# zhuzhui-2000/mobilesuperresolution

Measured on AMD Instinct MI355X. Metric: HR megapixels/sec (WDSR-B x4, 48x48 LR patches), full training step, higher is better.
Workload: dtype bf16; 1 GPU; WDSR-B x4, 16 blocks / 24 units, 48x48 LR patches, batch 32 per GPU, fwd+L1+bwd+Adam; global_batch=32, parallelism=dp1

## Files before the change

mobilesuperresolution_amd/csrc/sr_abi.hip:

```cpp
#include <algorithm>
#include <cmath>
#include "../../include/sr_hotpath.h"
#include "wdsr_block.h"
#include "wdsr_fwd_rs.h"
#include "wdsr_fwd_stream.h"
#include "wdsr_bwd_rs.h"
#include "wdsr_bwd_pair_lds.h"
#include "wdsr_wgrad_rs.h"
#include "wdsr_ends.h"
#include "wdsr_prep.h"
#include "conv3x3.h"
#include "conv64.h"
#include "conv64_bwd.h"
#include "vsr_recon.h"
#include "vsr_recon_bwd.h"
#include "mv_recon.h"
#include "spynet_conv.h"
#include "nas_block.h"
#include "nas_dw_lc.h"
#include "nas_bwd_fused.h"
#include "flow_warp.h"
#include "metrics.h"
#include "ssim.h"
#include "eval.h"
// ... 298 lines not shown
  if (dtype != SR_DTYPE_BF16) return -1;
  return dispatch_f(F, [&](auto d) {
    return launch_wgrad_saved<decltype(d)::F>(x, dy, tsave, dtsave, wblob, cinit, pa, pb, layers, wgs, N, H, W, x_ls, dy_ls, side_ls,
                                                  w_ls, c_ls, (hipStream_t)stream);
  });
}

extern "C" int sr_wdsr_block_slab_sizes(int F, int* slab_a, int* slab_b) {
  if (!slab_a || !slab_b) return -2;
  return dispatch_f(F, [&](auto d) {
    typedef BwdCfg<typename decltype(d)::Cfg> B;
    *slab_a = B::SLAB_A;
    *slab_b = B::SLAB_B;
    return 0;
  });
}

extern "C" int sr_wdsr_block_fwd(const void* x, void* y, const void* wblob, const float* cinit, int N, int H,
                                 int W, int F, int dtype, sr_stream_t stream) {
  if (!x || !y || !wblob || !cinit || N <= 0 || H <= 0 || W <= 0 || N > 65535) return -2;
  return dispatch_ft(F, dtype, [&](auto d, auto t) {
    return launch_block_fwd<decltype(t), decltype(d)::F>(x, y, wblob, cinit, N, H, W, (hipStream_t)stream);
  });
}

namespace {
template <typename E> dim3 tile_grid(int N, int H, int W, int* tiles_x) {
  *tiles_x = (W + E::TW - 1) / E::TW;
  return dim3(*tiles_x * ((H + E::TH - 1) / E::TH), N);
}
#define SR_DISPATCH_TF(CALL)                                                     \
  if (F == 24 && dtype == SR_DTYPE_BF16) { CALL(__bf16, 24) }                    \
  else if (F == 24 && dtype == SR_DTYPE_F32) { CALL(float, 24) }                 \
  else if (F == 32 && dtype == SR_DTYPE_BF16) { CALL(__bf16, 32) }               \
  else if (F == 32 && dtype == SR_DTYPE_F32) { CALL(float, 32) }                 \
  else return -1;
#define SR_DISPATCH_R(CALL, T, F_)                                               \
  if (R == 4) { CALL(T, F_, 4) } else if (R == 2) { CALL(T, F_, 2) } else if (R == 3) { CALL(T, F_, 3) } else return -1;
}

extern "C" int sr_head_fwd(const float* x, void* y, const void* wblob, float mean, int N, int H, int W, int F,
                           int dtype, sr_stream_t stream) {
  if (!x || !y || !wblob || N <= 0 || H <= 0 || W <= 0 || N > 65535) return -2;
  hipStream_t st = (hipStream_t)stream;
#define CALL(T, F_) { typedef EndsCfg<F_, 4> E; int tx; dim3 g = tile_grid<E>(N, H, W, &tx); \
    hipLaunchKernelGGL((sr_head_fwd_kernel<T, F_>), g, dim3(256), 0, st, x, (T*)y, (const T*)wblob, mean, H, W, tx); }
  SR_DISPATCH_TF(CALL)
#undef CALL
  SR_HIP_CHECK_LAUNCH();
  return 0;
}

extern "C" int sr_tail_fwd(const void* feat, const float* x, float* out, const void* wblob, float mean, int N,
                           int H, int W, int F, int R, int dtype, sr_stream_t stream) {
  if (!feat || !x || !out || !wblob || N <= 0 || H <= 0 || W <= 0 || N > 65535) return -2;
  hipStream_t st = (hipStream_t)stream;
#define CALLR(T, F_, R_) { typedef EndsCfg<F_, R_> E; int tx; dim3 g = tile_grid<E>(N, H, W, &tx); \
    hipLaunchKernelGGL((sr_tail_fwd_kernel<T, F_, R_>), g, dim3(SR_TAIL_FWD_THREADS), 0, st, (const T*)feat, x, out, (const T*)wblob, mean, H, W, tx); }
#define CALL(T, F_) SR_DISPATCH_R(CALLR, T, F_)
  SR_DISPATCH_TF(CALL)
#undef CALL
#undef CALLR
  SR_HIP_CHECK_LAUNCH();
  return 0;
}

namespace {
template <int LOSS>
int tail_bwd_data_t(const float* dout, const float* hr, float gscale, void* dfeat, const void* wblob, int N, int H, int W, int F,
                    int R, int dtype, hipStream_t st) {
  const LossIn li{hr, gscale};
#define CALLR(T, F_, R_) { typedef EndsCfg<F_, R_> E; int tx; dim3 g = tile_grid<E>(N, H, W, &tx); \
    hipLaunchKernelGGL((sr_tail_bwd_data_kernel<T, F_, R_, LOSS>), g, dim3(256), 0, st, dout, (T*)dfeat, (const T*)wblob, H, W, tx, li); }
#define CALL(T, F_) SR_DISPATCH_R(CALLR, T, F_)
  SR_DISPATCH_TF(CALL)
#undef CALL
#undef CALLR
  SR_HIP_CHECK_LAUNCH();
  return 0;
}
template <int LOSS>
int tail_wgrad_t(const float* dout, const float* hr, float gscale, float* loss_part, const void* feat, const float* x, float mean,
                 float* partial, int wgs, int N, int H, int W, int F, int R, int dtype, hipStream_t st) {
  const LossIn li{hr, gscale};
#define CALLR(T, F_, R_) { typedef EndsCfg<F_, R_> E; const int tx = (W + E::TW - 1) / E::TW, tpi = tx * ((H + E::TH - 1) / E::TH); \
    hipLaunchKernelGGL((sr_tail_wgrad_kernel<T, F_, R_, LOSS>), dim3(wgs), dim3(896), 0, st, dout, (const T*)feat, x, mean, partial, N, H, W, tx, tpi, li, loss_part); }
#define CALL(T, F_) SR_DISPATCH_R(CALLR, T, F_)
  SR_DISPATCH_TF(CALL)
#undef CALL
#undef CALLR
  SR_HIP_CHECK_LAUNCH();
  return 0;
}
template <int LOSS>
int tail_bwd_t(const float* dout, const float* hr, float gscale, float* loss_part, const void* feat, const float* x, float mean,
               const void* wblob, void* dfeat, float* partial, int wgs, int N, int H, int W, int F, int R, hipStream_t st) {
  const LossIn li{hr, gscale};
  typedef __bf16 TB;
#define CALLR(T, F_, R_) { typedef EndsCfg<F_, R_> E; const int tx = (W + E::TW - 1) / E::TW, tpi = tx * ((H + E::TH - 1) / E::TH); \
    hipLaunchKernelGGL((sr_tail_bwd_kernel<T, F_, R_, LOSS>), dim3(wgs), dim3(896), 0, st, dout, (const T*)feat, x, mean, (const T*)wblob, (T*)dfeat, partial, N, H, W, tx, tpi, li, loss_part); }
  if (F == 24) { SR_DISPATCH_R(CALLR, TB, 24) } else if (F == 32) { SR_DISPATCH_R(CALLR, TB, 32) } else return -1;
#undef CALLR
  SR_HIP_CHECK_LAUNCH();
  return 0;
}
}

extern "C" int sr_tail_bwd_data(const float* dout, void* dfeat, const void* wblob, int N, int H, int W, int F,
                                int R, int dtype, sr_stream_t stream) {
  if (!dout || !dfeat || !wblob || N <= 0 || H <= 0 || W <= 0 || N > 65535) return -2;
  return tail_bwd_data_t<0>(dout, nullptr, 0.f, dfeat, wblob, N, H, W, F, R, dtype, (hipStream_t)stream);
}

extern "C" int sr_tail_wgrad(const float* dout, const void* feat, const float* x, float mean, float* partial,
                             int wgs, int N, int H, int W, int F, int R, int dtype, sr_stream_t stream) {
  if (!dout || !feat || !x || !partial || wgs <= 0 || N <= 0 || H <= 0 || W <= 0) return -2;
  return tail_wgrad_t<0>(dout, nullptr, 0.f, nullptr, feat, x, mean, partial, wgs, N, H, W, F, R, dtype, (hipStream_t)stream);
}

extern "C" int sr_tail_bwd(const float* dout, const void* feat, const float* x, float mean, const void* wblob,
                          void* dfeat, float* partial, int wgs, int N, int H, int W, int F, int R, int dtype,
                          sr_stream_t stream) {
  if (!dout || !feat || !x || !wblob || !dfeat || !partial || wgs <= 0 || N <= 0 || H <= 0 || W <= 0) return -2;
  if (dtype != SR_DTYPE_BF16) return -1;
  return tail_bwd_t<0>(dout, nullptr, 0.f, nullptr, feat, x, mean, wblob, dfeat, partial, wgs, N, H, W, F, R, (hipStream_t)stream);
}

extern "C" int sr_tail_bwd_loss(const float* sr, const float* hr, int loss_kind, float gscale, float* loss_part, const void* feat,
                                const float* x, float mean, const void* wblob, void* dfeat, float* partial, int wgs, int N,
                                int H, int W, int F, int R, int dtype, sr_stream_t stream) {
  if (!sr || !hr || !loss_part || !feat || !x || !wblob || !dfeat || !partial || wgs <= 0 || N <= 0 || H <= 0 || W <= 0 || N > 65535)
    return -2;
  if (loss_kind != 1 && loss_kind != 2) return -1;
  hipStream_t st = (hipStream_t)stream;
  if (dtype == SR_DTYPE_BF16)
    return loss_kind == 1 ? tail_bwd_t<1>(sr, hr, gscale, loss_part, feat, x, mean, wblob, dfeat, partial, wgs, N, H, W, F, R, st)
                          : tail_bwd_t<2>(sr, hr, gscale, loss_part, feat, x, mean, wblob, dfeat, partial, wgs, N, H, W, F, R, st);
  int rc = loss_kind == 1 ? tail_bwd_data_t<1>(sr, hr, gscale, dfeat, wblob, N, H, W, F, R, dtype, st)
                          : tail_bwd_data_t<2>(sr, hr, gscale, dfeat, wblob, N, H, W, F, R, dtype, st);
  if (rc) return rc;
  return loss_kind == 1 ? tail_wgrad_t<1>(sr, hr, gscale, loss_part, feat, x, mean, partial, wgs, N, H, W, F, R, dtype, st)
                        : tail_wgrad_t<2>(sr, hr, gscale, loss_part, feat, x, mean, partial, wgs, N, H, W, F, R, dtype, st);
}

extern "C" int sr_tail_train(const float* hr, int loss_kind, float gscale, float* loss_part, const void* feat, const float* x,
                             float mean, const void* wblob, void* dfeat, float* partial, int wgs, int N, int H, int W, int F,
                             int R, int dtype, sr_stream_t stream) {
  if (!hr || !loss_part || !feat || !x || !wblob || !dfeat || !partial || wgs <= 0 || N <= 0 || H <= 0 || W <= 0 || N > 65535)
    return -2;
  if (dtype != SR_DTYPE_BF16 || R != 4 || (F != 24 && F != 32) || (loss_kind != 1 && loss_kind != 2)) return -1;
  hipStream_t st = (hipStream_t)stream;
  const LossIn li{hr, gscale};
  typedef __bf16 TB;
#define CALL(F_, LOSS) { typedef EndsCfg<F_, 4> E; const int tx = (W + E::TW - 1) / E::TW, tpi = tx * ((H + E::TH - 1) / E::TH); \
    hipLaunchKernelGGL((sr_tail_train_kernel<TB, F_, 4, LOSS>), dim3(wgs), dim3(896), 0, st, (const TB*)feat, x, mean, (const TB*)wblob, (TB*)dfeat, partial, N, H, W, tx, tpi, li, loss_part); }
  if (F == 24) { if (loss_kind == 1) CALL(24, 1) else CALL(24, 2) }
  else { if (loss_kind == 1) CALL(32, 1) else CALL(32, 2) }
#undef CALL
  SR_HIP_CHECK_LAUNCH();
  return 0;
}

extern "C" int sr_head_wgrad(const void* dy0, const float* x, float mean, float* partial, int wgs, int N, int H,
                             int W, int F, int dtype, sr_stream_t stream) {
  if (!dy0 || !x || !partial || wgs <= 0 || N <= 0 || H <= 0 || W <= 0) return -2;
  hipStream_t st = (hipStream_t)stream;
#define CALL(T, F_) { typedef EndsCfg<F_, 4> E; const int tx = (W + E::TW - 1) / E::TW, tpi = tx * ((H + E::TH - 1) / E::TH); \
    hipLaunchKernelGGL((sr_head_wgrad_kernel<T, F_>), dim3(wgs), dim3(576), 0, st, (const T*)dy0, x, mean, partial, N, H, W, tx, tpi); }
  SR_DISPATCH_TF(CALL)
#undef CALL
  SR_HIP_CHECK_LAUNCH();
  return 0;
}

namespace {
struct C3Grid { int tx, tpi; dim3 grid; };
inline C3Grid c3_grid(int N, int H, int W) {
  C3Grid g;
  g.tx = (W + C3Cfg::TW - 1) / C3Cfg::TW;
  g.tpi = g.tx * ((H + C3Cfg::TH - 1) / C3Cfg::TH);
  g.grid = dim3(g.tpi, N);
  return g;
}
template <typename T> C3WarpSrc<T> c3_warp_src(const sr_c3_warp_t* w) {
  C3WarpSrc<T> s{};
  if (w) { s.frame = w->frame; s.state = (const T*)w->state; s.flow = w->flow; s.frame_bs = w->frame_bs; s.flow_bs = w->flow_bs; s.x0_save = (T*)w->x0_save; }
  return s;
}
template <typename T>
int c3_fwd_t(const void* x, const void* res, void* y, const void* w, int N, int H, int W, int CI, int act, hipStream_t st,
             const sr_c3_warp_t* warp = nullptr, C3Dir dir = C3Dir{0, 0}) {
  const C3Grid g = c3_grid(N, H, W);
  const dim3 blk(64 * C3Cfg::NPT_O);
  const C3WarpSrc<T> ws = c3_warp_src<T>(warp);
#define L(CI_, ONES_, ACT_, ADD_) hipLaunchKernelGGL((c3_fwd_kernel<T, CI_, ONES_, ACT_, ADD_>), g.grid, blk, 0, st, (const T*)x, (const T*)res, (T*)y, (const T*)w, H, W, g.tx, ws, dir)
  if (warp) {
    if (CI != 32 || act != 2 || res) return -1;
    hipLaunchKernelGGL((c3_fwd_kernel<T, 32, 27, 2, false, true>), g.grid, blk, 0, st, (const T*)nullptr, (const T*)nullptr, (T*)y,
                       (const T*)w, H, W, g.tx, ws, dir);
  } else if (CI == 32 && act == 2 && !res) L(32, 27, 2, false);
  else if (CI == 24 && act == 2 && !res) L(24, 24, 2, false);
  else if (CI == 24 && act == 1 && !res) L(24, 24, 1, false);
  else if (CI == 24 && act == 0 && res) L(24, 24, 0, true);
  else if (CI == 24 && act == 0 && !res) L(24, 24, 0, false);
  else return -1;
#undef L
  SR_HIP_CHECK_LAUNCH();
  return 0;
}
template <typename T>
int c3_bwd_t(const void* dA, const void* A, const void* add, void* dx, const void* w, int N, int H, int W, int CI, int act,
             hipStream_t st, C3Dir dir = C3Dir{0, 0}) {
  const C3Grid g = c3_grid(N, H, W);
  const dim3 blk(64 * C3Cfg::NPT_O);
#define L(CI_, ACT_, ADD_) hipLaunchKernelGGL((c3_bwd_data_kernel<T, CI_, ACT_, ADD_>), g.grid, blk, 0, st, (const T*)dA, (const T*)A, (const T*)add, (T*)dx, (const T*)w, H, W, g.tx, dir)
  if (CI == 32 && act == 2 && !add) L(32, 2, false);
  else if (CI == 24 && act == 2 && !add) L(24, 2, false);
  else if (CI == 24 && act == 1 && add) L(24, 1, true);
  else if (CI == 24 && act == 1 && !add) L(24, 1, false);
  else if (CI == 24 && act == 0 && !add) L(24, 0, false);
  else return -1;
#undef L
  SR_HIP_CHECK_LAUNCH();
  return 0;
}
template <typename T>
int c3_wgrad_t(const void* x, const void* dA, const void* A, float* partial, int wgs, int N, int H, int W, int CI, int act,
               hipStream_t st, int layers = 1, long x_ls = 0, long d_ls = 0, long a_ls = 0, long p_ls = 0,
               const sr_c3_warp_t* warp = nullptr, int n_dir = 0) {
  const C3Grid g = c3_grid(N, H, W);
  const C3WarpSrc<T> ws = c3_warp_src<T>(warp);
#define L(CI_, ONES_, ACT_) hipLaunchKernelGGL((c3_wgrad_kernel<T, CI_, ONES_, ACT_>), dim3(wgs, layers), dim3(576), 0, st, (const T*)x, (const T*)dA, (const T*)A, partial, N, H, W, g.tx, g.tpi, x_ls, d_ls, a_ls, p_ls, ws, n_dir)
  if (warp) {
    if (CI != 32 || act != 2 || layers != 1) return -1;
    hipLaunchKernelGGL((c3_wgrad_kernel<T, 32, 27, 2, true>), dim3(wgs, 1), dim3(576), 0, st, (const T*)nullptr, (const T*)dA,
                       (const T*)A, partial, N, H, W, g.tx, g.tpi, x_ls, d_ls, a_ls, p_ls, ws, n_dir);
  } else if (CI == 32 && act == 2) L(32, 27, 2);
  else if (CI == 24 && act == 2) L(24, 24, 2);
  else if (CI == 24 && act == 1) L(24, 24, 1);
  else if (CI == 24 && act == 0) L(24, 24, 0);
  else return -1;
#undef L
  SR_HIP_CHECK_LAUNCH();
  return 0;
}
}

extern "C" int sr_c3_fwd(const void* x, const void* res, void* y, const void* wblob, int N, int H, int W, int CI,
                         int act, int dtype, sr_stream_t stream) {
  if (!x || !y || !wblob || N <= 0 || H <= 0 || W <= 0 || N > 65535) return -2;
  return dtype == SR_DTYPE_BF16 ? c3_fwd_t<__bf16>(x, res, y, wblob, N, H, W, CI, act, (hipStream_t)stream)
                                : c3_fwd_t<float>(x, res, y, wblob, N, H, W, CI, act, (hipStream_t)stream);
}
extern "C" int sr_c3_bwd_data(const void* dA, const void* A, const void* add, void* dx, const void* wblob, int N,
                              int H, int W, int CI, int act, int dtype, sr_stream_t stream) {
  if (!dA || !dx || !wblob || (act != 0 && !A) || N <= 0 || H <= 0 || W <= 0 || N > 65535) return -2;
  if (!A) A = dA;
  return dtype == SR_DTYPE_BF16 ? c3_bwd_t<__bf16>(dA, A, add, dx, wblob, N, H, W, CI, act, (hipStream_t)stream)
                                : c3_bwd_t<float>(dA, A, add, dx, wblob, N, H, W, CI, act, (hipStream_t)stream);
}
extern "C" int sr_c3_wgrad(const void* x, const void* dA, const void* A, float* partial, int wgs, int N, int H,
                           int W, int CI, int act, int dtype, sr_stream_t stream) {
  if (!x || !dA || !partial || (act != 0 && !A) || wgs <= 0 || N <= 0 || H <= 0 || W <= 0) return -2;
  if (!A) A = dA;
  return dtype == SR_DTYPE_BF16 ? c3_wgrad_t<__bf16>(x, dA, A, partial, wgs, N, H, W, CI, act, (hipStream_t)stream)
                                : c3_wgrad_t<float>(x, dA, A, partial, wgs, N, H, W, CI, act, (hipStream_t)stream);
}

template <typename T>
static int c3_trunk_fwd_t(const void* x0, const sr_c3_warp_t* warp, void* acts_, void* mids_, const void* blob_,
                          const long* boff, int nb, int N, int H, int W, int ci0, hipStream_t st, C3Dir dir) {
  const size_t act = (size_t)N * H * W * 24;
  T* acts = (T*)acts_; T* mids = (T*)mids_; const T* blob = (const T*)blob_;
  int rc;
  if ((rc = c3_fwd_t<T>(x0, nullptr, acts, blob + boff[0], N, H, W, ci0, 2, st, warp, dir))) return rc;
  for (int i = 0; i < nb; ++i) {
    if constexpr (sizeof(T) == 2) {
      const C3Grid g = c3_grid(N, H, W);
      if (i + 1 < nb) {
        hipLaunchKernelGGL((c3_resblock2_fwd_kernel<T>), g.grid, dim3(64 * C3Quad::NWAVES), 0, st, acts + i * act, mids + i * act,
                           acts + (i + 1) * act, mids + (i + 1) * act, acts + (i + 2) * act, blob, boff[1 + 2 * i], boff[2 + 2 * i],
                           boff[3 + 2 * i], boff[4 + 2 * i], H, W, g.tx, dir);
        SR_HIP_CHECK_LAUNCH();
        ++i;
        continue;
      }
      hipLaunchKernelGGL((c3_resblock_fwd_kernel<T>), g.grid, dim3(64 * C3Pair::NPT_H), 0, st, acts + i * act, mids + i * act,
                         acts + (i + 1) * act, blob + boff[1 + 2 * i], blob + boff[2 + 2 * i], H, W, g.tx, dir);
      SR_HIP_CHECK_LAUNCH();
      continue;
    }
    if ((rc = c3_fwd_t<T>(acts + i * act, nullptr, mids + i * act, blob + boff[1 + 2 * i], N, H, W, 24, 1, st, nullptr, dir))) return rc;
    if ((rc = c3_fwd_t<T>(mids + i * act, acts + i * act, acts + (i + 1) * act, blob + boff[2 + 2 * i], N, H, W, 24, 0, st, nullptr, dir)))
      return rc;
  }
  return 0;
}
template <typename T>
static int c3_trunk_bwd_t(const void* x0, const sr_c3_warp_t* warp, const void* acts_, const void* mids_, void* ga_, void* gt_,
                          const void* blob_, const long* boff, float* parts, void* dx0, const sr_c3_unpack_t* up, int nb,
                          int wgs, int N, int H, int W, int ci0, hipStream_t st, C3Dir dir) {
  const size_t act = (size_t)N * H * W * 24;
  const T* acts = (const T*)acts_; const T* mids = (const T*)mids_; const T* blob = (const T*)blob_;
  T* ga = (T*)ga_; T* gt = (T*)gt_;
  const long slot = (long)wgs * 9 * 1024;
  int rc;
  for (int i = nb - 1; i >= 0; --i) {
    if constexpr (sizeof(T) == 2) {
      const C3Grid g = c3_grid(N, H, W);
      hipLaunchKernelGGL((c3_resblock_bwd_data_kernel<T>), g.grid, dim3(64 * C3Pair::NPT_H), 0, st, ga + (i + 1) * act,
                         mids + i * act, gt + i * act, ga + i * act, blob + boff[1 + 2 * i], blob + boff[2 + 2 * i], H, W, g.tx, dir);
// ... 2183 lines not shown
```

mobilesuperresolution_amd/csrc/wdsr_ends.h:

```cpp
#pragma once
#include "wdsr_block.h"

template <int F_, int R_>
struct EndsCfg {
  static constexpr int F = F_, R = R_;
  static constexpr int CO = 3 * R * R, NT = (CO + 31) / 32, COP = (CO + 7) / 8 * 8, CC = COP / 8, FC = F / 8;
  static constexpr int KST = (9 * FC + 15 + 1) / 2, KSTB = (9 * CC + 1) / 2;
  static constexpr int TH = 12, TW = 24, HW = TW + 2, HH = TH + 2, NPXH = HW * HH, NPXH_PAD = (NPXH + 31) / 32 * 32;
  static constexpr int NPT_O = (TH / 4) * (TW / 8), NPXC = TH * TW;
  static constexpr int FT_ELEMS = (NPXH_PAD + 2) * F;
  static constexpr int DC_ELEMS = (NPXH_PAD + 2) * COP;
  static constexpr int DCC_ELEMS = (NPXC + 2) * COP;
  static constexpr int DYC_ELEMS = (NPXC + 2) * F;
  template <int P> struct Img {
    static constexpr int IW = TW + 2 * P, IH = TH + 2 * P, NPI = IW * IH, ELEMS = (NPI + 8) * 4;
  };
  static constexpr int TAIL_TILES = 14 * NT;
};

template <typename T> SR_DEV typename FragOf<T>::type lds_chunk_half(const T* img, int off) {
  typedef typename FragOf<T>::half_type HalfT;
  const HalfT lo = *reinterpret_cast<const HalfT*>(img + off);
  const HalfT hi = *reinterpret_cast<const HalfT*>(img + off + 4);
  typename FragOf<T>::type f;
// ... 324 lines not shown
      if (q < 9 * E::CC) {
        const int u = q / E::CC, c = q - u * E::CC;
        off = (hbase + (u / 3) * E::HW + (u % 3)) * E::COP + c * 8;
      }
      acc = mma16<T>(load_wfrag<T>(wt, s, lane), lds_chunk<T>(DC, off), acc);
    }
    const int Y = ty0 + oy, X = tx0 + ox;
    if (Y < H && X < W) {
      T* o = dfeat + (((size_t)n * H + Y) * W + X) * F;
#pragma unroll
      for (int g = 0; g < E::FC; ++g) stream_store(reinterpret_cast<HalfT*>(o + g * 8 + hh * 4), acc_group<T>(acc, g));
    }
  }
}


template <typename T, int F, int R, int LOSS = 0>
__global__ __launch_bounds__(896) void sr_tail_wgrad_kernel(const float* __restrict__ dout, const T* __restrict__ feat,
                                                            const float* __restrict__ ximg, float mean,
                                                            float* __restrict__ partial, int N, int H, int W,
                                                            int tiles_x, int tiles_per_img, LossIn li, float* __restrict__ loss_part) {
  typedef EndsCfg<F, R> E;
  typedef typename E::template Img<2> I;
  typedef typename FragOf<T>::type FragT;
  constexpr int NT = E::NT, NTHREADS = 896;
  __shared__ __attribute__((aligned(16))) T smem[E::DCC_ELEMS + E::FT_ELEMS + I::ELEMS];
  T* const DC = smem;
  T* const FT = DC + E::DCC_ELEMS;
  T* const XI = FT + E::FT_ELEMS;
  const int tid = threadIdx.x, lane = tid & 63, wave = tid >> 6;
  const bool is_tap = wave < 9;
  const int ty = is_tap ? wave / 3 : wave - 9, tx = is_tap ? wave % 3 : 0;

  f32x16 acc[NT];
#pragma unroll
  for (int i = 0; i < NT; ++i) acc[i] = zero16();
  float lsum = 0.f;

  SR_STAMP_DECL;
  SR_STAMP();
  for (int t = blockIdx.x; t < N * tiles_per_img; t += gridDim.x) {
    const int n = t / tiles_per_img, tile = t - n * tiles_per_img;
    const int ty0 = (tile / tiles_x) * E::TH, tx0 = (tile % tiles_x) * E::TW;
    __syncthreads();
    SR_STAMP();
    LossIn lin = li;
    lin.hr += LOSS ? (size_t)n * 3 * H * R * W * R : 0;
    stage_dconv<T, E, 0, NTHREADS, LOSS>(DC, dout + (size_t)n * 3 * H * R * W * R, H, W, ty0, tx0, tid, lin, &lsum);
    SR_STAMP();
    stage_halo<T, E, F, NTHREADS>(FT, feat + (size_t)n * H * W * F, H, W, ty0, tx0, tid);
    stage_img<T, E, 2, NTHREADS>(XI, ximg + (size_t)n * 3 * H * W, mean, H, W, ty0, tx0, tid);
    SR_STAMP();
    __syncthreads();
    SR_STAMP();
    constexpr int UNR = sizeof(T) == 2 ? 3 : 1;
#pragma unroll UNR
    for (int ot = 0; ot < E::NPT_O; ++ot) {
      const int toy = (ot / (E::TW / 8)) * 4, tox = (ot % (E::TW / 8)) * 8;
#pragma unroll
      for (int s = 0; s < 2; ++s) {
        FragT b;
        if (is_tap) b = tr_frag<T>(FT, s, lane, [=](int p) { return ((toy + (p >> 3) + ty) * E::HW + tox + (p & 7) + tx) * F; });
        else b = tr_frag<T>(XI, s, lane, [=](int p) { return ((toy + (p >> 3) + ty) * I::IW + tox + (p & 7)) * 4; });
#pragma unroll
        for (int ti = 0; ti < NT; ++ti) {
          const FragT a = tr_frag<T>(DC, s, lane, [=](int p) { return ((toy + (p >> 3)) * E::TW + tox + (p & 7)) * E::COP + 32 * ti; });
          acc[ti] = mma16<T>(a, b, acc[ti]);
        }
      }
    }
  }
  SR_STAMP();
  float* out = partial + (size_t)blockIdx.x * E::TAIL_TILES * 1024;
  const int gbase = is_tap ? (ty * 3 + tx) * NT : (9 + ty) * NT;
#pragma unroll
  for (int ti = 0; ti < NT; ++ti)
#pragma unroll
    for (int i = 0; i < 16; ++i) out[((gbase + ti) * 16 + i) * 64 + lane] = acc[ti][i];
  if constexpr (LOSS != 0) wg_sum_store<NTHREADS>(lsum, reinterpret_cast<float*>(smem), loss_part + blockIdx.x, tid);
  SR_STAMP();
}

template <typename T, int F>
__global__ __launch_bounds__(576) void sr_head_wgrad_kernel(const T* __restrict__ dy0, const float* __restrict__ ximg,
                                                            float mean, float* __restrict__ partial, int N, int H,
                                                            int W, int tiles_x, int tiles_per_img) {
  typedef EndsCfg<F, 4> E;
  typedef typename E::template Img<1> I;
  typedef typename FragOf<T>::type FragT;
  constexpr int NTHREADS = 576;
  constexpr int STAGE_BYTES = (E::DYC_ELEMS + I::ELEMS) * (int)sizeof(T);
  constexpr int SLAB_BYTES = 9 * 1024 * 4;
  constexpr int LDS_BYTES = STAGE_BYTES > SLAB_BYTES ? STAGE_BYTES : SLAB_BYTES;
  __shared__ __attribute__((aligned(16))) char smem_raw[LDS_BYTES];
  T* const DY = reinterpret_cast<T*>(smem_raw);
  T* const XI = DY + E::DYC_ELEMS;
  const int tid = threadIdx.x, lane = tid & 63, wave = tid >> 6;
  const int ky = wave / 3, grp = wave - ky * 3;
  f32x16 acc = zero16();
  for (int t = blockIdx.x; t < N * tiles_per_img; t += gridDim.x) {
    const int n = t / tiles_per_img, tile = t - n * tiles_per_img;
    const int ty0 = (tile / tiles_x) * E::TH, tx0 = (tile % tiles_x) * E::TW;
    __syncthreads();
    stage_core<T, E, F, NTHREADS>(DY, dy0 + (size_t)n * H * W * F, H, W, ty0, tx0, tid);
    stage_img<T, E, 1, NTHREADS>(XI, ximg + (size_t)n * 3 * H * W, mean, H, W, ty0, tx0, tid);
    __syncthreads();
#pragma unroll
    for (int k = 0; k < 3; ++k) {
      const int ot = grp + 3 * k;
      const int toy = (ot / (E::TW / 8)) * 4, tox = (ot % (E::TW / 8)) * 8;
#pragma unroll
      for (int s = 0; s < 2; ++s) {
        const FragT a = tr_frag<T>(DY, s, lane, [=](int p) { return ((toy + (p >> 3)) * E::TW + tox + (p & 7)) * F; });
        const FragT b = tr_frag<T>(XI, s, lane, [=](int p) { return ((toy + (p >> 3) + ky) * I::IW + tox + (p & 7)) * 4; });
        acc = mma16<T>(a, b, acc);
      }
    }
  }
  __syncthreads();
  float* slab = reinterpret_cast<float*>(smem_raw);
  slab_store_tile(slab, wave, acc, lane);
  __syncthreads();
  float* out = partial + (size_t)blockIdx.x * 3 * 1024;
  for (int i = tid; i < 3 * 1024; i += NTHREADS) {
    const int k = i >> 10, w = i & 1023;
    out[i] = slab[(3 * k) * 1024 + w] + slab[(3 * k + 1) * 1024 + w] + slab[(3 * k + 2) * 1024 + w];
  }
}

template <typename T, typename E, int UNRD, typename WS>
SR_DEV void tail_dfeat_tile(const T* DC, const WS& wsrc, T* __restrict__ dfeat, int n, int H, int W, int ty0, int tx0, int ot, int lane) {
  typedef typename FragOf<T>::half_type HalfT;
  const int r = lane & 31, hh = lane >> 5;
  const int oy = (ot / (E::TW / 8)) * 4 + (r >> 3), ox = (ot % (E::TW / 8)) * 8 + (r & 7);
  const int hbase = oy * E::HW + ox;
  f32x16 d = zero16();
#pragma unroll UNRD
  for (int s = 0; s < E::KSTB; ++s) {
    const int q = 2 * s + hh;
    int off = hbase * E::COP;
    if (q < 9 * E::CC) {
      const int u = q / E::CC, c = q - u * E::CC;
      off = (hbase + (u / 3) * E::HW + (u % 3)) * E::COP + c * 8;
    }
    d = mma16<T>(wsrc.get(s, lane), lds_chunk<T>(DC, off), d);
  }
  const int Y = ty0 + oy, X = tx0 + ox;
  if (Y < H && X < W) {
    T* o = dfeat + (((size_t)n * H + Y) * W + X) * E::F;
#pragma unroll
    for (int g = 0; g < E::FC; ++g) stream_store(reinterpret_cast<HalfT*>(o + g * 8 + hh * 4), acc_group<T>(d, g));
  }
}
template <typename T, typename E, int UNR>
SR_DEV void tail_wgrad_tile(const T* DC, const T* FT, const T* XI, f32x16 (&acc)[E::NT], bool is_tap, int ty, int tx, int lane) {
  typedef typename E::template Img<2> I;
  typedef typename FragOf<T>::type FragT;
#pragma unroll UNR
  for (int ot = 0; ot < E::NPT_O; ++ot) {
    const int toy = (ot / (E::TW / 8)) * 4, tox = (ot % (E::TW / 8)) * 8;
#pragma unroll
    for (int s = 0; s < 2; ++s) {
      FragT b;
      if (is_tap) b = tr_frag<T>(FT, s, lane, [=](int p) { return ((toy + (p >> 3) + ty) * E::HW + tox + (p & 7) + tx) * E::F; });
      else b = tr_frag<T>(XI, s, lane, [=](int p) { return ((toy + (p >> 3) + ty) * I::IW + tox + (p & 7)) * 4; });
#pragma unroll
      for (int ti = 0; ti < E::NT; ++ti) {
        const FragT a = tr_frag<T>(DC, s, lane, [=](int p) { return ((toy + (p >> 3) + 1) * E::HW + tox + (p & 7) + 1) * E::COP + 32 * ti; });
        acc[ti] = mma16<T>(a, b, acc[ti]);
      }
    }
  }
}
template <typename E>
SR_DEV void tail_slab_store(float* __restrict__ partial, const f32x16 (&acc)[E::NT], bool is_tap, int ty, int tx, int lane) {
  float* out = partial + (size_t)blockIdx.x * E::TAIL_TILES * 1024;
  const int gbase = is_tap ? (ty * 3 + tx) * E::NT : (9 + ty) * E::NT;
#pragma unroll
  for (int ti = 0; ti < E::NT; ++ti)
#pragma unroll
    for (int i = 0; i < 16; ++i) out[((gbase + ti) * 16 + i) * 64 + lane] = acc[ti][i];
}
template <typename E, int LOSS> struct TailBwdUnroll {
  static constexpr int UNRD = (E::NT > 1 && E::F > 24) ? 3 : E::KSTB;
  static constexpr int UNR = (E::NT > 1 || (LOSS != 0 && E::R == 2)) ? 1 : 3;
};

template <typename T, int F, int R, int LOSS = 0>
__global__ __launch_bounds__(896) void sr_tail_bwd_kernel(const float* __restrict__ dout, const T* __restrict__ feat,
                                                          const float* __restrict__ ximg, float mean,
                                                          const T* __restrict__ wblob, T* __restrict__ dfeat,
                                                          float* __restrict__ partial, int N, int H, int W, int tiles_x,
                                                          int tiles_per_img, LossIn li, float* __restrict__ loss_part) {
  typedef EndsCfg<F, R> E;
  typedef typename E::template Img<2> I;
  typedef typename FragOf<T>::type FragT;
  typedef typename FragOf<T>::half_type HalfT;
  static_assert(sizeof(T) == 2, "bf16 only");
  constexpr int NT = E::NT, NTHREADS = 896;
  __shared__ __attribute__((aligned(16))) T smem[E::DC_ELEMS + E::FT_ELEMS + I::ELEMS + E::KSTB * 512];
  T* const DC = smem;
  T* const FT = DC + E::DC_ELEMS;
  T* const XI = FT + E::FT_ELEMS;
  T* const WL = XI + I::ELEMS;
  const int tid = threadIdx.x, lane = tid & 63, wave = tid >> 6, r = lane & 31, hh = lane >> 5;
  const bool is_tap = wave < 9;
  const int ty = is_tap ? wave / 3 : wave - 9, tx = is_tap ? wave % 3 : 0;
  stage_weights<T, NTHREADS>(WL, wblob + (size_t)E::NT * E::KST * 512, E::KSTB, tid);
  WSrc<T, true> wsrc;
  wsrc.p = WL;

  f32x16 acc[NT];
#pragma unroll
  for (int i = 0; i < NT; ++i) acc[i] = zero16();
  __shared__ float lsum_lds[LOSS ? NTHREADS : 1];
  if constexpr (LOSS != 0) lsum_lds[tid] = 0.f;

  for (int t = blockIdx.x; t < N * tiles_per_img; t += gridDim.x) {
    const int n = t / tiles_per_img, tile = t - n * tiles_per_img;
    const int ty0 = (tile / tiles_x) * E::TH, tx0 = (tile % tiles_x) * E::TW;
    __syncthreads();
    LossIn lin = li;
    lin.hr += LOSS ? (size_t)n * 3 * H * R * W * R : 0;
    {
      float lsum = 0.f;
      stage_dconv<T, E, 1, NTHREADS, LOSS>(DC, dout + (size_t)n * 3 * H * R * W * R, H, W, ty0, tx0, tid, lin, &lsum);
      if constexpr (LOSS != 0) lsum_lds[tid] += lsum;
    }
    stage_halo<T, E, F, NTHREADS>(FT, feat + (size_t)n * H * W * F, H, W, ty0, tx0, tid);
    stage_img<T, E, 2, NTHREADS>(XI, ximg + (size_t)n * 3 * H * W, mean, H, W, ty0, tx0, tid);
    __syncthreads();
    if (wave < E::NPT_O) {
      const int ot = wave;
      const int oy = (ot / (E::TW / 8)) * 4 + (r >> 3), ox = (ot % (E::TW / 8)) * 8 + (r & 7);
      const int hbase = oy * E::HW + ox;
      f32x16 d = zero16();
      constexpr int UNRD = (NT > 1 && F > 24) ? 3 : E::KSTB;
#pragma unroll UNRD
      for (int s = 0; s < E::KSTB; ++s) {
        const int q = 2 * s + hh;
        int off = hbase * E::COP;
        if (q < 9 * E::CC) {
          const int u = q / E::CC, c = q - u * E::CC;
          off = (hbase + (u / 3) * E::HW + (u % 3)) * E::COP + c * 8;
        }
        d = mma16<T>(wsrc.get(s, lane), lds_chunk<T>(DC, off), d);
      }
      const int Y = ty0 + oy, X = tx0 + ox;
      if (Y < H && X < W) {
        T* o = dfeat + (((size_t)n * H + Y) * W + X) * F;
#pragma unroll
        for (int g = 0; g < E::FC; ++g) stream_store(reinterpret_cast<HalfT*>(o + g * 8 + hh * 4), acc_group<T>(d, g));
      }
    }
    constexpr int UNR = (NT > 1 || (LOSS != 0 && R == 2) || (R == 3 && F > 24)) ? 1 : 3;
#pragma unroll UNR
    for (int ot = 0; ot < E::NPT_O; ++ot) {
      const int toy = (ot / (E::TW / 8)) * 4, tox = (ot % (E::TW / 8)) * 8;
#pragma unroll
      for (int s = 0; s < 2; ++s) {
        FragT b;
        if (is_tap) b = tr_frag<T>(FT, s, lane, [=](int p) { return ((toy + (p >> 3) + ty) * E::HW + tox + (p & 7) + tx) * F; });
        else b = tr_frag<T>(XI, s, lane, [=](int p) { return ((toy + (p >> 3) + ty) * I::IW + tox + (p & 7)) * 4; });
#pragma unroll
        for (int ti = 0; ti < NT; ++ti) {
          const FragT a = tr_frag<T>(DC, s, lane, [=](int p) { return ((toy + (p >> 3) + 1) * E::HW + tox + (p & 7) + 1) * E::COP + 32 * ti; });
          acc[ti] = mma16<T>(a, b, acc[ti]);
        }
      }
    }
  }
  float* out = partial + (size_t)blockIdx.x * E::TAIL_TILES * 1024;
  const int gbase = is_tap ? (ty * 3 + tx) * NT : (9 + ty) * NT;
#pragma unroll
  for (int ti = 0; ti < NT; ++ti)
#pragma unroll
    for (int i = 0; i < 16; ++i) out[((gbase + ti) * 16 + i) * 64 + lane] = acc[ti][i];
  if constexpr (LOSS != 0) wg_sum_store<NTHREADS>(lsum_lds[tid], reinterpret_cast<float*>(smem), loss_part + blockIdx.x, tid);
}

template <typename T, int F, int R, int LOSS>
__global__ __launch_bounds__(896) void sr_tail_train_kernel(const T* __restrict__ feat, const float* __restrict__ ximg, float mean,
                                                            const T* __restrict__ wblob, T* __restrict__ dfeat,
                                                            float* __restrict__ partial, int N, int H, int W, int tiles_x,
                                                            int tiles_per_img, LossIn li, float* __restrict__ loss_part) {
  typedef EndsCfg<F, R> E;
  typedef typename E::template Img<2> I;
  typedef typename E::template Img<3> I3;
  typedef typename FragOf<T>::type FragT;
  typedef typename FragOf<T>::half_type HalfT;
  static_assert(sizeof(T) == 2 && R == 4 && LOSS != 0 && E::COP == E::CO, "bf16, x4, with the loss");
  constexpr int NT = E::NT, NTHREADS = 896;
  constexpr int NPT_H = E::NPXH_PAD / 32;
  static_assert(NPT_H * 64 <= NTHREADS, "one wave per forward pixel tile");
  constexpr int HW2 = E::TW + 4, NPX2 = HW2 * (E::TH + 4);
  constexpr int FT2_ELEMS = NPX2 * F, FW_ELEMS = NT * E::KST * 512;
  constexpr int FWD_ELEMS = FW_ELEMS + FT2_ELEMS + I3::ELEMS;
  constexpr int TERM_ELEMS = E::NPXC * E::CO * 2;
  constexpr int BWD_ELEMS = E::DC_ELEMS + TERM_ELEMS;
  constexpr int U_ELEMS = FWD_ELEMS > BWD_ELEMS ? FWD_ELEMS : BWD_ELEMS;
  __shared__ __attribute__((aligned(16))) T smem[E::FT_ELEMS + I::ELEMS + E::KSTB * 512 + U_ELEMS];
  T* const FT = smem;
  T* const XI = FT + E::FT_ELEMS;
  T* const WL = XI + I::ELEMS;
  T* const DC = WL + E::KSTB * 512;
  float* const TERM = reinterpret_cast<float*>(DC + E::DC_ELEMS);
  T* const FW = DC;
  T* const FT2 = FW + FW_ELEMS;
  constexpr int XI3_0 = FT2_ELEMS;
  const int tid = threadIdx.x, lane = tid & 63, wave = tid >> 6, r = lane & 31, hh = lane >> 5;
  const bool is_tap = wave < 9;
  const int ty = is_tap ? wave / 3 : wave - 9, tx = is_tap ? wave % 3 : 0;
  stage_weights<T, NTHREADS>(WL, wblob + (size_t)E::NT * E::KST * 512, E::KSTB, tid);
  WSrc<T, true> wsrc, wfwd;
  wsrc.p = WL;
  wfwd.p = FW;

  f32x16 acc[NT];
#pragma unroll
  for (int i = 0; i < NT; ++i) acc[i] = zero16();
  __shared__ float lsum_lds[NTHREADS];
  lsum_lds[tid] = 0.f;

  const int p = wave * 32 + r;
  const bool fwd_wave = wave < NPT_H;
  constexpr int NG = E::CO / 8;

  for (int t = blockIdx.x; t < N * tiles_per_img; t += gridDim.x) {
    const int n = t / tiles_per_img, tile = t - n * tiles_per_img;
    const int ty0 = (tile / tiles_x) * E::TH, tx0 = (tile % tiles_x) * E::TW;
    int p_t = p;
    asm volatile("" : "+v"(p_t));
    const int pp = (fwd_wave && p_t < E::NPXH) ? p_t : 0;
    const int py = pp / E::HW, px = pp - py * E::HW;
    const bool core = py >= 1 && py <= E::TH && px >= 1 && px <= E::TW;
    const int Y = ty0 - 1 + py, X = tx0 - 1 + px;
    const bool live = fwd_wave && p < E::NPXH && Y >= 0 && Y < H && X >= 0 && X < W;
    const float* const hr = li.hr + (size_t)n * 3 * H * R * W * R;
    const unsigned hrw = (unsigned)W * R, plane = (unsigned)H * R * hrw;
    const unsigned hoff = ((unsigned)Y * R) * hrw + (unsigned)X * R + (hh ? hrw : 0u);
    float touch = 0.f;
    if (live) {
#pragma unroll
      for (int k = 0; k < NG; ++k) touch += hr[hoff + (k >> 1) * plane + (k & 1) * 2 * hrw];
    }
    __syncthreads();
    int tid_t = tid;
    asm volatile("" : "+v"(tid_t));
    stage_weights<T, NTHREADS>(FW, wblob, NT * E::KST, tid);
    stage_rows<T, F, HW2, NPX2, NPX2, NTHREADS>(FT2, feat + (size_t)n * H * W * F, H, W, ty0 - 2, tx0 - 2, tid_t);
    stage_img<T, E, 3, NTHREADS>(FT2 + XI3_0, ximg + (size_t)n * 3 * H * W, mean, H, W, ty0, tx0, tid_t);
    stage_halo<T, E, F, NTHREADS>(FT, feat + (size_t)n * H * W * F, H, W, ty0, tx0, tid_t);
    stage_img<T, E, 2, NTHREADS>(XI, ximg + (size_t)n * 3 * H * W, mean, H, W, ty0, tx0, tid_t);
    __syncthreads();
    f32x16 facc[NT];
    if (fwd_wave) {
      int lane_f = lane;
      asm volatile("" : "+v"(lane_f));
      const int hh_f = lane_f >> 5, hbase = py * HW2 + px;
#pragma unroll
      for (int ti = 0; ti < NT; ++ti) facc[ti] = zero16();
      const int fbase = hbase * F, xbase = XI3_0 + (py * I3::IW + px) * 4;
      auto chunk_off = [&](int q) {
        if (q < 9 * E::FC) {
          const int tap = q / E::FC, c = q - tap * E::FC;
          return fbase + ((tap / 3) * HW2 + (tap % 3)) * F + c * 8;
        }
        int qs = q - 9 * E::FC;
        if (qs >= 15) qs = 0;
        const int ky = qs / 3, m = qs - ky * 3;
        return xbase + (ky * I3::IW + 2 * m) * 4;
      };
#pragma unroll
      for (int s = 0; s < E::KST; ++s) {
        const int off = hh_f ? chunk_off(2 * s + 1) : chunk_off(2 * s);
        const FragT b = 2 * s + 1 < 9 * E::FC ? lds_chunk<T>(FT2, off) : lds_chunk_half<T>(FT2, off);
#pragma unroll
        for (int ti = 0; ti < NT; ++ti) facc[ti] = mma16<T>(wfwd.get(ti * E::KST + s, lane_f), b, facc[ti]);
      }
    }
    asm volatile("" :: "v"(touch));
    f32x4 hv[NG];
    if (live) {
#pragma unroll
      for (int k = 0; k < NG; ++k)
        hv[k] = *reinterpret_cast<const f32x4*>(hr + (hoff + (k >> 1) * plane + (k & 1) * 2 * hrw));
    } else {
#pragma unroll
      for (int k = 0; k < NG; ++k) hv[k] = f32x4{0.f, 0.f, 0.f, 0.f};
    }
    __syncthreads();
    if (fwd_wave) {
#pragma unroll
      for (int k = 0; k < NG; ++k) {
        const int ti = k >> 2, g = k & 3, ch0 = 8 * k + 4 * hh;
        HalfT dv;
        f32x4 tv;
#pragma unroll
        for (int j = 0; j < 4; ++j) {
          float term = 0.f;
          const float gj = live ? loss_grad<LOSS>(facc[ti][4 * g + j], hv[k][j], li.gscale, term) : 0.f;
          dv[j] = (T)gj;
          tv[j] = term;
        }
        *reinterpret_cast<HalfT*>(DC + p * E::COP + ch0) = dv;
        if (live && core) *reinterpret_cast<f32x4*>(TERM + ((py - 1) * E::TW + px - 1) * E::CO + ch0) = tv;
      }
    } else if (wave == NPT_H) {
      constexpr int NCH = 2 * E::COP / 8;
      FragT z;
#pragma unroll
      for (int j = 0; j < 8; ++j) z[j] = (T)0.f;
      if (lane < NCH) *reinterpret_cast<FragT*>(DC + E::NPXH_PAD * E::COP + lane * 8) = z;
    }
    __syncthreads();
    {
      constexpr int ROWS = 3 * R, TOTAL = (E::NPXH_PAD + 2) * ROWS, ITER = (TOTAL + NTHREADS - 1) / NTHREADS;
      float lsum = 0.f;
      int tid_l = tid;
      asm volatile("" : "+v"(tid_l));
#pragma unroll
      for (int it = 0; it < ITER; ++it) {
        const int idx = tid_l + it * NTHREADS;
        const int q = idx / ROWS, cr = idx - q * ROWS;
        if (q < E::NPXH) {
          const int qy = q / E::HW, qx = q - qy * E::HW;
          if (qy >= 1 && qy <= E::TH && qx >= 1 && qx <= E::TW && ty0 - 1 + qy < H && tx0 - 1 + qx < W) {
            const f32x4 tv = *reinterpret_cast<const f32x4*>(TERM + ((qy - 1) * E::TW + qx - 1) * E::CO + cr * R);
#pragma unroll
            for (int j = 0; j < R; ++j) lsum += tv[j];
          }
        }
      }
      lsum_lds[tid] += lsum;
    }
    typedef TailBwdUnroll<E, LOSS> U;
    int lane_d = lane;
    asm volatile("" : "+v"(lane_d));
    if (wave < E::NPT_O) tail_dfeat_tile<T, E, U::UNRD>(DC, wsrc, dfeat, n, H, W, ty0, tx0, wave, lane_d);
    tail_wgrad_tile<T, E, U::UNR>(DC, FT, XI, acc, is_tap, ty, tx, lane_d);
  }
  tail_slab_store<E>(partial, acc, is_tap, ty, tx, lane);
  wg_sum_store<NTHREADS>(lsum_lds[tid], reinterpret_cast<float*>(smem), loss_part + blockIdx.x, tid);
}
```

Before: 3500 HR-Mpix/s.

## Reuse forward-staged tiles for tail wgrad and add one-tile-per-workgroup specialization

The tail training kernel no longer stages a separate halo feature tile and padded image for the weight-gradient pass. Instead it reads offset views into the wider forward-stage buffers (FT2 and the pad-3 image). This removes redundant global loads and LDS writes and shrinks LDS use. A new ONE template path, chosen when the grid covers every tile, drops the loop-top barrier, the asm register pinning and the per-thread LDS loss accumulator. It also adds timing stamp macros and hard-codes view origins that must match the staging layouts.

```diff
diff --git a/mobilesuperresolution_amd/csrc/sr_abi.hip b/mobilesuperresolution_amd/csrc/sr_abi.hip
--- a/mobilesuperresolution_amd/csrc/sr_abi.hip
+++ b/mobilesuperresolution_amd/csrc/sr_abi.hip
@@ -474,11 +474,13 @@
   hipStream_t st = (hipStream_t)stream;
   const LossIn li{hr, gscale};
   typedef __bf16 TB;
+#define LAUNCH(F_, LOSS, ONE) hipLaunchKernelGGL((sr_tail_train_kernel<TB, F_, 4, LOSS, ONE>), dim3(wgs), dim3(896), 0, st, (const TB*)feat, x, mean, (const TB*)wblob, (TB*)dfeat, partial, N, H, W, tx, tpi, li, loss_part)
 #define CALL(F_, LOSS) { typedef EndsCfg<F_, 4> E; const int tx = (W + E::TW - 1) / E::TW, tpi = tx * ((H + E::TH - 1) / E::TH); \
-    hipLaunchKernelGGL((sr_tail_train_kernel<TB, F_, 4, LOSS>), dim3(wgs), dim3(896), 0, st, (const TB*)feat, x, mean, (const TB*)wblob, (TB*)dfeat, partial, N, H, W, tx, tpi, li, loss_part); }
+    if ((long)wgs >= (long)N * tpi) LAUNCH(F_, LOSS, true); else LAUNCH(F_, LOSS, false); }
   if (F == 24) { if (loss_kind == 1) CALL(24, 1) else CALL(24, 2) }
   else { if (loss_kind == 1) CALL(32, 1) else CALL(32, 2) }
 #undef CALL
+#undef LAUNCH
   SR_HIP_CHECK_LAUNCH();
   return 0;
 }
diff --git a/mobilesuperresolution_amd/csrc/wdsr_ends.h b/mobilesuperresolution_amd/csrc/wdsr_ends.h
--- a/mobilesuperresolution_amd/csrc/wdsr_ends.h
+++ b/mobilesuperresolution_amd/csrc/wdsr_ends.h
@@ -500,17 +500,21 @@
     for (int g = 0; g < E::FC; ++g) stream_store(reinterpret_cast<HalfT*>(o + g * 8 + hh * 4), acc_group<T>(d, g));
   }
 }
-template <typename T, typename E, int UNR>
+template <typename E, int PF, int PX> struct tail_view_origin {
+  static constexpr int FT = (PF - 1) * (E::TW + 2 * PF + 1) * E::F, XI = (PX - 2) * (E::template Img<PX>::IW + 1) * 4;
+};
+template <typename T, typename E, int UNR, int PF = 1, int PX = 2>
 SR_DEV void tail_wgrad_tile(const T* DC, const T* FT, const T* XI, f32x16 (&acc)[E::NT], bool is_tap, int ty, int tx, int lane) {
-  typedef typename E::template Img<2> I;
+  typedef typename E::template Img<PX> I;
   typedef typename FragOf<T>::type FragT;
+  constexpr int FW_ = E::TW + 2 * PF;
 #pragma unroll UNR
   for (int ot = 0; ot < E::NPT_O; ++ot) {
     const int toy = (ot / (E::TW / 8)) * 4, tox = (ot % (E::TW / 8)) * 8;
 #pragma unroll
     for (int s = 0; s < 2; ++s) {
       FragT b;
-      if (is_tap) b = tr_frag<T>(FT, s, lane, [=](int p) { return ((toy + (p >> 3) + ty) * E::HW + tox + (p & 7) + tx) * E::F; });
+      if (is_tap) b = tr_frag<T>(FT, s, lane, [=](int p) { return ((toy + (p >> 3) + ty) * FW_ + tox + (p & 7) + tx) * E::F; });
       else b = tr_frag<T>(XI, s, lane, [=](int p) { return ((toy + (p >> 3) + ty) * I::IW + tox + (p & 7)) * 4; });
 #pragma unroll
       for (int ti = 0; ti < E::NT; ++ti) {
@@ -627,13 +631,16 @@
   if constexpr (LOSS != 0) wg_sum_store<NTHREADS>(lsum_lds[tid], reinterpret_cast<float*>(smem), loss_part + blockIdx.x, tid);
 }
 
-template <typename T, int F, int R, int LOSS>
+template <bool ONE> SR_DEV int tile_local(int v) {
+  if constexpr (!ONE) asm volatile("" : "+v"(v));
+  return v;
+}
+template <typename T, int F, int R, int LOSS, bool ONE>
 __global__ __launch_bounds__(896) void sr_tail_train_kernel(const T* __restrict__ feat, const float* __restrict__ ximg, float mean,
                                                             const T* __restrict__ wblob, T* __restrict__ dfeat,
                                                             float* __restrict__ partial, int N, int H, int W, int tiles_x,
                                                             int tiles_per_img, LossIn li, float* __restrict__ loss_part) {
   typedef EndsCfg<F, R> E;
-  typedef typename E::template Img<2> I;
   typedef typename E::template Img<3> I3;
   typedef typename FragOf<T>::type FragT;
   typedef typename FragOf<T>::half_type HalfT;
@@ -643,19 +650,20 @@
   static_assert(NPT_H * 64 <= NTHREADS, "one wave per forward pixel tile");
   constexpr int HW2 = E::TW + 4, NPX2 = HW2 * (E::TH + 4);
   constexpr int FT2_ELEMS = NPX2 * F, FW_ELEMS = NT * E::KST * 512;
-  constexpr int FWD_ELEMS = FW_ELEMS + FT2_ELEMS + I3::ELEMS;
   constexpr int TERM_ELEMS = E::NPXC * E::CO * 2;
   constexpr int BWD_ELEMS = E::DC_ELEMS + TERM_ELEMS;
-  constexpr int U_ELEMS = FWD_ELEMS > BWD_ELEMS ? FWD_ELEMS : BWD_ELEMS;
-  __shared__ __attribute__((aligned(16))) T smem[E::FT_ELEMS + I::ELEMS + E::KSTB * 512 + U_ELEMS];
-  T* const FT = smem;
-  T* const XI = FT + E::FT_ELEMS;
-  T* const WL = XI + I::ELEMS;
+  constexpr int U_ELEMS = FW_ELEMS > BWD_ELEMS ? FW_ELEMS : BWD_ELEMS;
+  constexpr int LDS_ELEMS = FT2_ELEMS + I3::ELEMS + E::KSTB * 512 + U_ELEMS;
+  constexpr int NLSUM = ONE ? 1 : NTHREADS;
+  static_assert(LDS_ELEMS * sizeof(T) + NLSUM * sizeof(float) <= 160 * 1024, "the LDS a workgroup may take");
+  static_assert(FT2_ELEMS % 8 == 0 && I3::ELEMS % 8 == 0, "16-byte aligned regions");
+  __shared__ __attribute__((aligned(16))) T smem[LDS_ELEMS];
+  T* const FT2 = smem;
+  constexpr int XI3_0 = FT2_ELEMS;
+  T* const WL = FT2 + FT2_ELEMS + I3::ELEMS;
   T* const DC = WL + E::KSTB * 512;
   float* const TERM = reinterpret_cast<float*>(DC + E::DC_ELEMS);
   T* const FW = DC;
-  T* const FT2 = FW + FW_ELEMS;
-  constexpr int XI3_0 = FT2_ELEMS;
   const int tid = threadIdx.x, lane = tid & 63, wave = tid >> 6, r = lane & 31, hh = lane >> 5;
   const bool is_tap = wave < 9;
   const int ty = is_tap ? wave / 3 : wave - 9, tx = is_tap ? wave % 3 : 0;
@@ -667,8 +675,11 @@
   f32x16 acc[NT];
 #pragma unroll
   for (int i = 0; i < NT; ++i) acc[i] = zero16();
-  __shared__ float lsum_lds[NTHREADS];
-  lsum_lds[tid] = 0.f;
+  __shared__ float lsum_lds[NLSUM];
+  float lsum_one = 0.f;
+  if constexpr (!ONE) lsum_lds[tid] = 0.f;
+  SR_STAMP_DECL;
+  SR_STAMP();
 
   const int p = wave * 32 + r;
   const bool fwd_wave = wave < NPT_H;
@@ -677,8 +688,7 @@
   for (int t = blockIdx.x; t < N * tiles_per_img; t += gridDim.x) {
     const int n = t / tiles_per_img, tile = t - n * tiles_per_img;
     const int ty0 = (tile / tiles_x) * E::TH, tx0 = (tile % tiles_x) * E::TW;
-    int p_t = p;
-    asm volatile("" : "+v"(p_t));
+    const int p_t = tile_local<ONE>(p);
     const int pp = (fwd_wave && p_t < E::NPXH) ? p_t : 0;
     const int py = pp / E::HW, px = pp - py * E::HW;
     const bool core = py >= 1 && py <= E::TH && px >= 1 && px <= E::TW;
@@ -692,19 +702,16 @@
 #pragma unroll
       for (int k = 0; k < NG; ++k) touch += hr[hoff + (k >> 1) * plane + (k & 1) * 2 * hrw];
     }
-    __syncthreads();
-    int tid_t = tid;
-    asm volatile("" : "+v"(tid_t));
+    if constexpr (!ONE) __syncthreads();
+    const int tid_t = tile_local<ONE>(tid);
     stage_weights<T, NTHREADS>(FW, wblob, NT * E::KST, tid);
     stage_rows<T, F, HW2, NPX2, NPX2, NTHREADS>(FT2, feat + (size_t)n * H * W * F, H, W, ty0 - 2, tx0 - 2, tid_t);
     stage_img<T, E, 3, NTHREADS>(FT2 + XI3_0, ximg + (size_t)n * 3 * H * W, mean, H, W, ty0, tx0, tid_t);
-    stage_halo<T, E, F, NTHREADS>(FT, feat + (size_t)n * H * W * F, H, W, ty0, tx0, tid_t);
-    stage_img<T, E, 2, NTHREADS>(XI, ximg + (size_t)n * 3 * H * W, mean, H, W, ty0, tx0, tid_t);
     __syncthreads();
+    SR_STAMP();
     f32x16 facc[NT];
     if (fwd_wave) {
-      int lane_f = lane;
-      asm volatile("" : "+v"(lane_f));
+      const int lane_f = tile_local<ONE>(lane);
       const int hh_f = lane_f >> 5, hbase = py * HW2 + px;
 #pragma unroll
       for (int ti = 0; ti < NT; ++ti) facc[ti] = zero16();
@@ -727,6 +734,7 @@
         for (int ti = 0; ti < NT; ++ti) facc[ti] = mma16<T>(wfwd.get(ti * E::KST + s, lane_f), b, facc[ti]);
       }
     }
+    SR_STAMP();
     asm volatile("" :: "v"(touch));
     f32x4 hv[NG];
     if (live) {
@@ -762,11 +770,11 @@
       if (lane < NCH) *reinterpret_cast<FragT*>(DC + E::NPXH_PAD * E::COP + lane * 8) = z;
     }
     __syncthreads();
+    SR_STAMP();
     {
       constexpr int ROWS = 3 * R, TOTAL = (E::NPXH_PAD + 2) * ROWS, ITER = (TOTAL + NTHREADS - 1) / NTHREADS;
       float lsum = 0.f;
-      int tid_l = tid;
-      asm volatile("" : "+v"(tid_l));
+      const int tid_l = tile_local<ONE>(tid);
 #pragma unroll
       for (int it = 0; it < ITER; ++it) {
         const int idx = tid_l + it * NTHREADS;
@@ -780,14 +788,19 @@
           }
         }
       }
-      lsum_lds[tid] += lsum;
+      if constexpr (ONE) lsum_one = lsum;
+      else lsum_lds[tid] += lsum;
     }
     typedef TailBwdUnroll<E, LOSS> U;
-    int lane_d = lane;
-    asm volatile("" : "+v"(lane_d));
+    const int lane_d = tile_local<ONE>(lane);
     if (wave < E::NPT_O) tail_dfeat_tile<T, E, U::UNRD>(DC, wsrc, dfeat, n, H, W, ty0, tx0, wave, lane_d);
-    tail_wgrad_tile<T, E, U::UNR>(DC, FT, XI, acc, is_tap, ty, tx, lane_d);
+    SR_STAMP();
+    typedef tail_view_origin<E, 2, 3> V;
+    tail_wgrad_tile<T, E, U::UNR, 2, 3>(DC, FT2 + V::FT, FT2 + XI3_0 + V::XI, acc, is_tap, ty, tx, lane_d);
+    SR_STAMP();
+    if constexpr (ONE) break;
   }
   tail_slab_store<E>(partial, acc, is_tap, ty, tx, lane);
-  wg_sum_store<NTHREADS>(lsum_lds[tid], reinterpret_cast<float*>(smem), loss_part + blockIdx.x, tid);
-}
+  wg_sum_store<NTHREADS>(ONE ? lsum_one : lsum_lds[ONE ? 0 : tid], reinterpret_cast<float*>(smem), loss_part + blockIdx.x, tid);
+  SR_STAMP();
+}
```

Result: faster. 3550 HR-Mpix/s, median of 6 (+1.4%).
